# Kodifly/FAST-LIO-SAM_GPS

Measured on AMD Instinct MI355X. Metric: scans/sec (100k-pt scan vs N-pt map) + ms/IESKF-iteration, 1 GPU, higher is better.
Workload: dtype f32/f64; 1 GPU; C3: 131072-pt livox scan vs 5000000-pt map grown by 20 scans (map_incremental), max_iteration=3 (<=4 h-evals/scan); scan_points=131072, map_points=5000000, resident_scans=8, parallelism=replicas x1 (front end does not shard)

## Files before the change

fast-lio-sam_gps_amd/csrc/ieskf.cpp:

```cpp
#include "ieskf.hpp"

#include <chrono>
#include <cmath>
#include <cstring>

namespace lio {
namespace host {

namespace {

constexpr double kTol = 1e-11;
constexpr double kGravLen = 98090.0 / 10000.0;
constexpr int kSO3[2] = {3, 6};
constexpr int kS2 = 21;

Quat qmul(const Quat& a, const Quat& b) {
    return {a.w * b.w - a.x * b.x - a.y * b.y - a.z * b.z, a.w * b.x + a.x * b.w + a.y * b.z - a.z * b.y,
            a.w * b.y + a.y * b.w + a.z * b.x - a.x * b.z, a.w * b.z + a.z * b.w + a.x * b.y - a.y * b.x};
}

Quat qexp(const double* v, double h) {
    const double nrm = std::sqrt(v[0] * v[0] + v[1] * v[1] + v[2] * v[2]);
    if (nrm < kTol) return {1.0, h * v[0], h * v[1], h * v[2]};
    const double a = h * nrm, s = std::sin(a) / nrm;
// ... 126 lines not shown
    qlog(qmul(oc, x.offR), d + 6);
    for (int i = 0; i < 3; ++i) {
        d[9 + i] = x.offT[i] - y.offT[i];
        d[12 + i] = x.vel[i] - y.vel[i];
        d[15 + i] = x.bg[i] - y.bg[i];
        d[18 + i] = x.ba[i] - y.ba[i];
    }
    s2_minus(x.grav, y.grav, d + 21);
}

void boxplus(State& x, const double* d) {
    for (int i = 0; i < 3; ++i) x.pos[i] += d[i];
    x.rot = qmul(x.rot, qexp(d + 3, 0.5));
    x.offR = qmul(x.offR, qexp(d + 6, 0.5));
    for (int i = 0; i < 3; ++i) {
        x.offT[i] += d[9 + i];
        x.vel[i] += d[12 + i];
        x.bg[i] += d[15 + i];
        x.ba[i] += d[18 + i];
    }
    s2_plus(x.grav, d + 21);
}

bool lu_inverse(Mat& A, int n) {
    std::vector<int> piv(n);
    Mat LU = A;
    for (int k = 0; k < n; ++k) {
        int p = k;
        double best = std::fabs(LU[(size_t)k * n + k]);
        for (int r = k + 1; r < n; ++r) {
            const double v = std::fabs(LU[(size_t)r * n + k]);
            if (v > best) {
                best = v;
                p = r;
            }
        }
        piv[k] = p;
        if (best == 0.0) return false;
        if (p != k)
            for (int c = 0; c < n; ++c) std::swap(LU[(size_t)k * n + c], LU[(size_t)p * n + c]);
        const double inv = 1.0 / LU[(size_t)k * n + k];
        for (int r = k + 1; r < n; ++r) {
            const double f = (LU[(size_t)r * n + k] *= inv);
            if (f != 0.0)
                for (int c = k + 1; c < n; ++c) LU[(size_t)r * n + c] -= f * LU[(size_t)k * n + c];
        }
    }
    Mat X((size_t)n * n, 0.0);
    std::vector<double> col(n);
    for (int j = 0; j < n; ++j) {
        for (int i = 0; i < n; ++i) col[i] = (i == j) ? 1.0 : 0.0;
        for (int k = 0; k < n; ++k)
            if (piv[k] != k) std::swap(col[k], col[piv[k]]);
        for (int i = 0; i < n; ++i) {
            double s = col[i];
            for (int k = 0; k < i; ++k) s -= LU[(size_t)i * n + k] * col[k];
            col[i] = s;
        }
        for (int i = n - 1; i >= 0; --i) {
            double s = col[i];
            for (int k = i + 1; k < n; ++k) s -= LU[(size_t)i * n + k] * col[k];
            col[i] = s / LU[(size_t)i * n + i];
        }
        for (int i = 0; i < n; ++i) X[(size_t)i * n + j] = col[i];
    }
    A.swap(X);
    return true;
}

void rows_apply(Mat& Dst, const Mat& Src, int stride, int idx, const double* T, int d, int ncols) {
    double tmp[3];
    for (int c = 0; c < ncols; ++c) {
        for (int r = 0; r < d; ++r) {
            double s = 0;
            for (int k = 0; k < d; ++k) s += T[r * d + k] * Src[(size_t)(idx + k) * stride + c];
            tmp[r] = s;
        }
        for (int r = 0; r < d; ++r) Dst[(size_t)(idx + r) * stride + c] = tmp[r];
    }
}
void cols_apply(Mat& M, int nrows, int stride, int idx, const double* T, int d) {
    double tmp[3];
    for (int r = 0; r < nrows; ++r) {
        double* row = &M[(size_t)r * stride + idx];
        for (int c = 0; c < d; ++c) {
            double s = 0;
            for (int k = 0; k < d; ++k) s += row[k] * T[c * d + k];
            tmp[c] = s;
        }
// ... 13 lines not shown

}

void quat_to_mat(const Quat& q, double R[9]) {
    const double tx = 2 * q.x, ty = 2 * q.y, tz = 2 * q.z;
    const double twx = tx * q.w, twy = ty * q.w, twz = tz * q.w;
    const double txx = tx * q.x, txy = ty * q.x, txz = tz * q.x;
    const double tyy = ty * q.y, tyz = tz * q.y, tzz = tz * q.z;
    R[0] = 1 - (tyy + tzz);
    R[1] = txy - twz;
    R[2] = txz + twy;
    R[3] = txy + twz;
    R[4] = 1 - (txx + tzz);
    R[5] = tyz - twx;
    R[6] = txz - twy;
    R[7] = tyz + twx;
    R[8] = 1 - (txx + tyy);
}

int update_iterated(State& x, Mat& P, double R, int max_iter, double epsi, const HModelFn& hfn, IeskfResult& out) {
    using clk = std::chrono::steady_clock;
    const State x_prop = x;
    const Mat P_prop = P;
    Mat K_x((size_t)N * N, 0.0), Mm(36);
    double K_h[N], dx_new[N], dxu[N];
    bool converge = true;
    int t = 0;
    HModel hm;
    out = IeskfResult{};
    double solve_s = 0.0;
    for (int i = -1; i < max_iter; ++i) {
        const bool want_rows_hint = false;
        ++out.h_evals;
        if (converge) ++out.knn_calls;
        int rc = hfn(x, converge, want_rows_hint, hm);
        if (rc != 0) return rc;
        const int dof = (int)hm.sums[27];
        out.n_eff = dof;
        out.res_mean = dof > 0 ? hm.sums[28] / dof : 0.0;
        if (dof < 1) continue;
        if (dof < N && hm.rows.size() != (size_t)7 * dof) {
            rc = hfn(x, false, true, hm);
            if (rc != 0) return rc;
        }
        const auto t0 = clk::now();
        double dx[N];
        boxminus(x, x_prop, dx);
        std::memcpy(dx_new, dx, sizeof(dx));
// ... 13 lines not shown
            const double v1 = T2[2] * dx_new[kS2] + T2[3] * dx_new[kS2 + 1];
            dx_new[kS2] = v0;
            dx_new[kS2 + 1] = v1;
            rows_apply(P, P, N, kS2, T2, 2, N);
            cols_apply(P, N, N, kS2, T2, 2);
        }
        std::fill(K_x.begin(), K_x.end(), 0.0);
        if (N > dof) {
            const double* H = hm.rows.data();
            Mat PHt((size_t)N * dof);
            for (int r = 0; r < N; ++r)
                for (int m = 0; m < dof; ++m) {
                    double s = 0;
                    for (int c = 0; c < 6; ++c) s += P[(size_t)r * N + c] * H[7 * m + c];
                    PHt[(size_t)r * dof + m] = s;
                }
            Mat S((size_t)dof * dof);
            for (int a = 0; a < dof; ++a)
                for (int b = 0; b < dof; ++b) {
                    double s = 0;
                    for (int c = 0; c < 6; ++c) s += H[7 * a + c] * PHt[(size_t)c * dof + b];
                    S[(size_t)a * dof + b] = s / R + (a == b ? 1.0 : 0.0);
                }
            if (!lu_inverse(S, dof)) return -4;
            for (int r = 0; r < N; ++r) {
                double kh = 0;
                double kx[6] = {0, 0, 0, 0, 0, 0};
                for (int b = 0; b < dof; ++b) {
                    double s = 0;
                    for (int a = 0; a < dof; ++a) s += PHt[(size_t)r * dof + a] * S[(size_t)a * dof + b];
                    const double k = s / R;
                    kh += k * H[7 * b + 6];
                    for (int c = 0; c < 6; ++c) kx[c] += k * H[7 * b + c];
                }
                K_h[r] = kh;
                for (int c = 0; c < 6; ++c) K_x[(size_t)r * N + c] = kx[c];
            }
        } else {
            double HTH[36];
            unpack_hth(hm.sums, HTH);
            double PR[N * 6];
            for (int r = 0; r < N; ++r)
                for (int m = 0; m < 6; ++m) PR[r * 6 + m] = P[(size_t)r * N + m] / R;
            Mm.assign(36, 0.0);
            for (int a = 0; a < 6; ++a)
                for (int b = 0; b < 6; ++b) {
                    double s = 0;
                    for (int m = 0; m < 6; ++m) s += HTH[6 * a + m] * PR[m * 6 + b];
                    Mm[(size_t)a * 6 + b] = s + (a == b ? 1.0 : 0.0);
                }
            if (!lu_inverse(Mm, 6)) return -4;
            for (int r = 0; r < N; ++r) {
                double q[6];
                for (int c = 0; c < 6; ++c) {
                    double s = 0;
                    for (int m = 0; m < 6; ++m) s += PR[r * 6 + m] * Mm[(size_t)m * 6 + c];
                    q[c] = s;
                }
                double kh = 0;
                for (int c = 0; c < 6; ++c) kh += q[c] * hm.sums[21 + c];
                K_h[r] = kh;
                for (int c = 0; c < 6; ++c) {
                    double s = 0;
                    for (int m = 0; m < 6; ++m) s += q[m] * HTH[6 * m + c];
                    K_x[(size_t)r * N + c] = s;
                }
            }
        }
        for (int r = 0; r < N; ++r) {
            double s = 0;
            for (int c = 0; c < 6; ++c) s += (K_x[(size_t)r * N + c] - (r == c ? 1.0 : 0.0)) * dx_new[c];
            if (r >= 6) s += -dx_new[r];
            dxu[r] = K_h[r] + s;
        }
        boxplus(x, dxu);
        converge = true;
        for (int r = 0; r < N; ++r)
            if (std::fabs(dxu[r]) > epsi) {
                converge = false;
                break;
            }
        if (converge) ++t;
        if (!t && i == max_iter - 2) converge = true;
        if (t > 1 || i == max_iter - 1) {
            Mat L = P;
            for (int idx : kSO3) {
                const M3 At = transpose(a_matrix(dxu + idx));
                rows_apply(L, P, N, idx, At.a, 3, N);
                rows_apply(K_x, K_x, N, idx, At.a, 3, 12);
                cols_apply(L, N, N, idx, At.a, 3);
                cols_apply(P, N, N, idx, At.a, 3);
            }
            {
                double T2[4];
                s2_jac(x.grav, x_prop.grav, dxu + kS2, T2);
                rows_apply(L, P, N, kS2, T2, 2, N);
                rows_apply(K_x, K_x, N, kS2, T2, 2, 12);
                cols_apply(L, N, N, kS2, T2, 2);
                cols_apply(P, N, N, kS2, T2, 2);
            }
            Mat Pn((size_t)N * N);
            for (int r = 0; r < N; ++r)
                for (int c = 0; c < N; ++c) {
                    double s = 0;
                    for (int m = 0; m < 6; ++m) s += K_x[(size_t)r * N + m] * P[(size_t)m * N + c];
                    Pn[(size_t)r * N + c] = L[(size_t)r * N + c] - s;
                }
            P.swap(Pn);
            out.converged = t > 1 ? 1 : 0;
            solve_s += std::chrono::duration<double>(clk::now() - t0).count();
            break;
        }
        solve_s += std::chrono::duration<double>(clk::now() - t0).count();
    }
    out.solve_ms = solve_s * 1e3;
    return 0;
}

}
}
```

fast-lio-sam_gps_amd/csrc/lio_capi_online.hpp:

```cpp
#pragma once
#include <atomic>
#include <cmath>

#include "lio_capi_util.hpp"
#include "lio_mapupd.hpp"

struct lio_map : lio::capi::Handle {
    uint64_t version = 0;
    std::atomic<int> n_ctx{0};
    lio_map_params p{};
    lio::GridBuf grid;
    lio::MapUpdBuf upd;
    float* d_xyz = nullptr;
    int64_t xyz_cap = 0;
    int64_t n = 0;
    int32_t* d_qidx = nullptr;
    int64_t qidx_cap = 0;
    float* d_qd2 = nullptr;
    int64_t qd2_cap = 0;
};

namespace lio::capi {
struct EventPair {
    hipEvent_t a = nullptr, b = nullptr;
// ... 1 lines not shown
}

struct lio_ctx {
    lio_map* map = nullptr;
    double last_launch_ms = 0.0, last_wait_ms = 0.0;
    lio_match_params p{};
    int64_t n = 0, cap = 0;
    float* d_body = nullptr;
    const float* body_ext = nullptr;
    int32_t* d_nn = nullptr;
    float4* d_planes = nullptr;
    uint8_t* d_sel = nullptr;
    double* d_partials = nullptr;
    int64_t part_cap = 0;
    double* d_sums = nullptr;
    double* h_sums = nullptr;
    double* h_sums_dev = nullptr;
    unsigned long long seq = 0;
    double* d_rows = nullptr;
    int64_t rows_cap = 0;
    int64_t* d_nrows = nullptr;
    lio_pose last_pose{};
    lio_pose knn_pose{};
    int* d_far_list = nullptr;
    int* d_far_count = nullptr;
    unsigned* d_done = nullptr;
    float* d_far_d = nullptr;
    int* d_far_id = nullptr;
    float* d_d5 = nullptr;
    float* d_dbg = nullptr;
    int64_t dbg_cap = 0;
    bool have_eval = false;
    bool knn_valid = false;
    uint64_t knn_map_version = 0;
    bool timing = false;
    lio_kernel_timing tm{};
    lio::capi::EventPair ev_main, ev_fin;
    hipEvent_t ev_marks[8] = {};
    lio::FilterBuf filt;
    float* d_raw = nullptr;
    int64_t raw_cap = 0;
    float* d_rec = nullptr;
    int64_t rec_cap = 0;
    lio::ImuPose* d_poses = nullptr;
    int64_t poses_cap = 0;
    float seed_scale = 1.0f;
    int64_t undist_n = -1;
    int undist_stride = 0;
    float* d_kf = nullptr;
    int64_t kf_cap = 0;
};
// ... 56 lines not shown
```

fast-lio-sam_gps_amd/csrc/lio_capi_scan.cpp:

```cpp
#include <algorithm>
#include <chrono>
#include <cmath>
#include <cstring>
#include <string>

#include "ieskf.hpp"
#include "lio_capi_online.hpp"

using namespace lio::capi;

static void ctx_free(lio_ctx& c) {
    lio::dev_free(&c.d_body, &c.d_nn, &c.d_planes, &c.d_sel, &c.d_partials, &c.d_sums, &c.d_rows, &c.d_nrows,
                  &c.d_far_list, &c.d_far_count, &c.d_far_d, &c.d_far_id, &c.d_done, &c.d_d5, &c.d_dbg, &c.d_raw,
                  &c.d_rec, &c.d_poses, &c.d_kf);
    lio::host_free(&c.h_sums);
    for (hipEvent_t* e : {&c.ev_main.a, &c.ev_main.b, &c.ev_fin.a, &c.ev_fin.b})
        if (*e) (void)hipEventDestroy(*e);
    for (hipEvent_t e : c.ev_marks)
        if (e) (void)hipEventDestroy(e);
    lio::filter_free(c.filt);
}

int lio::capi::ctx_reserve(lio_ctx* c, int64_t n) {
    if (n > c->cap || !c->d_body) {
        const int64_t cap = std::max<int64_t>(n, c->cap + c->cap / 2);
        c->cap = 0;
        if (lio::dev_alloc_all({lio::dev_req(c->d_body, cap * 3), lio::dev_req(c->d_nn, cap * 5),
                                lio::dev_req(c->d_planes, cap), lio::dev_req(c->d_sel, cap + 64),
                                lio::dev_req(c->d_far_list, cap), lio::dev_req(c->d_far_d, cap * 5),
                                lio::dev_req(c->d_far_id, cap * 5), lio::dev_req(c->d_d5, cap)}))
            return fail(LIO_ERR_NOMEM, "scan buffers: hipMalloc failed");
        c->cap = cap;
    }
    int rc = grow(&c->d_partials, c->part_cap, (int64_t)lio::match_blocks((int)n) * 32 + 32);
    if (rc) return rc;
    c->n = n;
    c->body_ext = nullptr;
    c->have_eval = false;
    c->knn_valid = false;
    return LIO_OK;
}

extern "C" {

int lio_ctx_create(lio_map* m, const lio_match_params* p, lio_ctx** out) {
    if (!m || !out) return fail(LIO_ERR_ARG, "bad arguments");
    HIP_TRY(hipSetDevice(m->dev));
    auto* c = new lio_ctx();
    c->map = m;
    ++m->n_ctx;
    if (p)
        c->p = *p;
    else
        c->p = lio_match_params{5.0f, 0.1f, 0.9, 0.9};
    if (hipMalloc(&c->d_sums, 32 * sizeof(double)) != hipSuccess ||
        hipHostMalloc(&c->h_sums, 40 * sizeof(double), hipHostMallocMapped | hipHostMallocCoherent) != hipSuccess ||
        hipHostGetDevicePointer(reinterpret_cast<void**>(&c->h_sums_dev), c->h_sums, 0) != hipSuccess ||
// ... 45 lines not shown
}

int lio_scan_bind_device(lio_ctx* c, const float* d_body, int64_t n) {
    if (!c || n < 0 || (n > 0 && !d_body) || n >= (int64_t)1 << 30) return fail(LIO_ERR_ARG, "lio_scan_bind_device: bad arguments");
    HIP_TRY(hipSetDevice(c->map->dev));
    int rc = ctx_reserve(c, n);
    if (rc) return rc;
    c->body_ext = n ? d_body : nullptr;
    return LIO_OK;
}

static_assert(sizeof(lio_pose) == sizeof(lio::PoseArg), "lio_pose / PoseArg layout");

static lio::MatchArgs make_args(lio_ctx* c, const lio_pose& pose_in) {
    lio::MatchArgs a{};
    const lio_pose pose = filled(pose_in);
    std::memcpy(&a.pose, &pose, sizeof(lio::PoseArg));
    a.grid = lio::grid_view(c->map->grid);
    a.body = body_ptr(c);
    a.map_by_id = c->map->grid.by_id;
    a.nn_idx = c->d_nn;
    a.nn_d5 = c->d_d5;
    a.seed_scale = c->seed_scale;
    {
        const lio_pose pk = filled(c->knn_pose);
        std::memcpy(&a.pose_knn, &pk, sizeof(lio::PoseArg));
        double R[9], RL[9];
        quat_to_mat(pk.q, R);
        quat_to_mat(pk.q_LI, RL);
        for (int r = 0; r < 3; ++r) {
            for (int k = 0; k < 3; ++k)
                a.knn_M[4 * r + k] =
                    (float)(R[3 * r] * RL[k] + R[3 * r + 1] * RL[3 + k] + R[3 * r + 2] * RL[6 + k]);
            a.knn_M[4 * r + 3] =
                (float)(R[3 * r] * pk.t_LI[0] + R[3 * r + 1] * pk.t_LI[1] + R[3 * r + 2] * pk.t_LI[2] + pk.t[r]);
        }
    }
    a.planes = c->d_planes;
    a.sel = c->d_sel;
    a.partials = c->d_partials;
    a.n = (int)c->n;
    a.max_shell = (int)std::ceil(std::sqrt((double)c->p.knn_range_sq) / a.grid.cell) + 1;
    a.dbg = nullptr;
    a.sums_out = c->h_sums_dev;
    a.seq_out = reinterpret_cast<unsigned long long*>(c->h_sums_dev + 32);
    a.seq = 0;
    a.far_list = c->d_far_list;
    a.far_count = c->d_far_count;
    a.done_count = c->d_done;
    a.far_d = c->d_far_d;
    a.far_id = c->d_far_id;
    a.range_sq = c->p.knn_range_sq;
    a.plane_thr = c->p.plane_thr;
    a.s_coef = c->p.s_coef;
    a.s_gate = c->p.s_gate;
    return a;
}

static void accum_event(EventPair& e, int64_t& launches, double& ms) {
    float t = 0.f;
    if (hipEventElapsedTime(&t, e.a, e.b) == hipSuccess) {
        ms += t;
        ++launches;
    }
}

static uint64_t mix64(uint64_t z) {
    z = (z ^ (z >> 30)) * 0xbf58476d1ce4e5b9ull;
    z = (z ^ (z >> 27)) * 0x94d049bb133111ebull;
    return z ^ (z >> 31);
}

static bool read_result(const lio_ctx* c, unsigned long long seq, double* sums) {
    const volatile uint64_t* w = reinterpret_cast<const volatile uint64_t*>(c->h_sums);
    if (w[32] != seq) return false;
    uint64_t h = 0, bits[LIO_SUMS_LEN];
    for (int l = 0; l < LIO_SUMS_LEN; ++l) {
        bits[l] = w[l];
        h ^= mix64(bits[l] ^ ((uint64_t)l * 0x9e3779b97f4a7c15ull));
    }
    if ((h ^ mix64(seq)) != w[33]) return false;
    std::memcpy(sums, bits, sizeof(bits));
    return true;
}

static int wait_result(lio_ctx* c, unsigned long long seq, double* sums) {
    for (uint64_t it = 0;; ++it) {
        if (read_result(c, seq, sums)) return LIO_OK;
        if ((it & 255) == 255) {
            const hipError_t e = hipStreamQuery(c->map->st);
            if (e != hipSuccess && e != hipErrorNotReady)
                return fail(LIO_ERR_HIP, std::string("lio_match: ") + hipGetErrorString(e));
            if (e == hipSuccess && !read_result(c, seq, sums))
                return fail(LIO_ERR_HIP, "lio_match: evaluation produced no result");
        }
    }
}

static int match_impl(lio_ctx* c, const lio_pose* pose_in, int redo_knn, double* sums);

int lio_match(lio_ctx* c, const lio_pose* pose_in, int redo_knn, double* sums) {
    if (!c || !pose_in || !sums) return fail(LIO_ERR_ARG, "lio_match: bad arguments");
    return match_impl(c, pose_in, redo_knn, sums);
}

static int match_impl(lio_ctx* c, const lio_pose* pose_in, int redo_knn, double* sums) {
    const lio_pose pose_f = filled(*pose_in);
    const lio_pose* pose = &pose_f;
    if (c->map->grid.n_ids == 0) return fail(LIO_ERR_STATE, "lio_match: map is empty (call lio_map_build)");
    if (!redo_knn && !c->knn_valid) return fail(LIO_ERR_STATE, "lio_match: redo_knn=0 before any kNN evaluation");
    if (!redo_knn && c->knn_map_version != c->map->version)
        return fail(LIO_ERR_STATE, "lio_match: redo_knn=0 but the map changed since this scan's kNN evaluation");
    HIP_TRY(hipSetDevice(c->map->dev));
    hipStream_t st = c->map->st;
    lio::MatchArgs a = make_args(c, *pose);
    if (c->map->n == 0 && c->n > 0) {
        HIP_TRY(hipMemsetAsync(c->d_nn, 0xff, c->n * 5 * sizeof(int32_t), st));
        HIP_TRY(hipMemsetAsync(c->d_sel, 0, c->n, st));
        HIP_TRY(hipStreamSynchronize(st));
    }
    if (c->n == 0 || c->map->n == 0) {
        std::memset(sums, 0, LIO_SUMS_LEN * sizeof(double));
        c->last_pose = *pose;
        c->have_eval = true;
        c->knn_valid = true;
        c->knn_map_version = c->map->version;
        c->knn_pose = *pose;
        return LIO_OK;
    }
    a.seq = ++c->seq;
    a.prior = (redo_knn && c->knn_valid && c->knn_map_version == c->map->version) ? 1 : 0;
    const auto t0 = std::chrono::steady_clock::now();
    if (c->timing) HIP_TRY(hipEventRecord(c->ev_main.a, st));
    lio::launch_h_model(a, redo_knn != 0, st, c->timing ? c->ev_marks : nullptr);
    if (c->timing) HIP_TRY(hipEventRecord(c->ev_main.b, st));
    HIP_TRY(hipGetLastError());
    const auto t1 = std::chrono::steady_clock::now();
    int rc = wait_result(c, a.seq, sums);
    if (rc) return rc;
    const auto t2 = std::chrono::steady_clock::now();
    c->last_launch_ms = std::chrono::duration<double, std::milli>(t1 - t0).count();
    c->last_wait_ms = std::chrono::duration<double, std::milli>(t2 - t1).count();
    if (c->timing) {
        HIP_TRY(hipEventSynchronize(c->ev_main.b));
        if (redo_knn) {
            const double before = c->tm.near_ms + c->tm.far_ms + c->tm.plane_ms;
            EventPair n{c->ev_marks[0], c->ev_marks[1]}, f{c->ev_marks[2], c->ev_marks[3]},
                p{c->ev_marks[4], c->ev_marks[5]};
            accum_event(n, c->tm.near_launches, c->tm.near_ms);
            if (a.max_shell > 1) accum_event(f, c->tm.far_launches, c->tm.far_ms);
            accum_event(p, c->tm.plane_launches, c->tm.plane_ms);
            c->tm.knn_ms += (c->tm.near_ms + c->tm.far_ms + c->tm.plane_ms) - before;
            ++c->tm.knn_launches;
        } else {
            EventPair r{c->ev_marks[6], c->ev_marks[7]};
            accum_event(r, c->tm.reuse_launches, c->tm.reuse_ms);
        }
    }
    c->last_pose = *pose;
    c->have_eval = true;
    if (redo_knn) {
        c->knn_valid = true;
        c->knn_map_version = c->map->version;
        c->knn_pose = *pose;
    }
    return LIO_OK;
}

int lio_ctx_knn_stats(lio_ctx* c, const lio_pose* pose, double* sums, int32_t* stats3) {
    if (!c || !pose || !sums || !stats3) return fail(LIO_ERR_ARG, "lio_ctx_knn_stats: bad arguments");
    if (c->map->n == 0) return fail(LIO_ERR_STATE, "lio_ctx_knn_stats: map is empty");
    HIP_TRY(hipSetDevice(c->map->dev));
    hipStream_t st = c->map->st;
    if (c->n == 0) return LIO_OK;
    static_assert(sizeof(int) == sizeof(float), "the debug scratch holds either");
    int rc = grow(&c->d_dbg, c->dbg_cap, c->n * 3);
    if (rc) return rc;
    lio::MatchArgs a = make_args(c, *pose);
    a.dbg = reinterpret_cast<int*>(c->d_dbg);
    a.seq = ++c->seq;
    lio::launch_h_model(a, true, st);
    hipError_t e2 = hipMemcpyAsync(stats3, c->d_dbg, c->n * 3 * sizeof(int), hipMemcpyDeviceToHost, st);
    hipError_t e3 = hipStreamSynchronize(st);
    if (e2 != hipSuccess || e3 != hipSuccess) return fail(LIO_ERR_HIP, "lio_ctx_knn_stats failed");
    rc = wait_result(c, a.seq, sums);
    if (rc) return rc;
    c->last_pose = *pose;
    c->knn_pose = *pose;
    c->have_eval = true;
    c->knn_valid = true;
    c->knn_map_version = c->map->version;
    return LIO_OK;
}

int lio_ctx_get_knn_pose(lio_ctx* c, lio_pose* out) {
    if (!c || !out) return fail(LIO_ERR_ARG, "bad arguments");
    if (!c->knn_valid) return fail(LIO_ERR_STATE, "lio_ctx_get_knn_pose: no kNN evaluation");
    *out = c->knn_pose;
    return LIO_OK;
}

int lio_map_incremental(lio_ctx* c, const lio_pose* pose, double filter_size_map, lio_incremental_stats* st) {
    if (!c || !pose || !(filter_size_map > 0.0)) return fail(LIO_ERR_ARG, "lio_map_incremental: bad arguments");
    if (c->n > 0 && !c->knn_valid && c->map->n > 0)
        return fail(LIO_ERR_STATE, "lio_map_incremental: no kNN evaluation for this scan (Nearest_Points)");
    if (c->n > 0 && c->map->n > 0 && c->knn_map_version != c->map->version)
        return fail(LIO_ERR_STATE, "lio_map_incremental: the map changed since this scan's kNN evaluation");
    lio_map* m = c->map;
// ... 200 lines not shown
```

fast-lio-sam_gps_amd/csrc/lio_dev.hpp:

```cpp
#pragma once
#include <hip/hip_runtime.h>
#include <stdint.h>

namespace lio {

constexpr int kNone = 0x7fffffff;

struct GridDev {
    const float4* pts;
    const uint32_t* start;
    const uint2* rng;
    float ox, oy, oz;
    float cell, inv_cell;
    float margin;
    int nx, ny, nz;
};

struct PoseArg {
    double R[9];
    double t[3];
    double RLI[9];
    double tLI[3];
    double q[4];
    double qLI[4];
// ... 122 lines not shown
    float g = fmaxf(fmaxf(lo - q, q - hi), 0.f);
    return g * g;
}

template <int OFF>
__device__ __forceinline__ uint32_t partner_u32(uint32_t v) {
    if constexpr (OFF == 1) return (uint32_t)__builtin_amdgcn_update_dpp((int)v, (int)v, 0xb1, 0xf, 0xf, false);
    else if constexpr (OFF == 2) return (uint32_t)__builtin_amdgcn_update_dpp((int)v, (int)v, 0x4e, 0xf, 0xf, false);
    else if constexpr (OFF == 4) return (uint32_t)__builtin_amdgcn_update_dpp((int)v, (int)v, 0x141, 0xf, 0xf, false);
    else return (uint32_t)__shfl_xor((int)v, OFF, 64);
}
template <int OFF>
__device__ __forceinline__ float partner_f(float v) {
    return __uint_as_float(partner_u32<OFF>(__float_as_uint(v)));
}

template <int G, int OFF = 1>
__device__ __forceinline__ float group_min(float v) {
    if constexpr (OFF >= G) {
        return v;
    } else {
        v = fminf(v, partner_f<OFF>(v));
        return group_min<G, 2 * OFF>(v);
    }
}

template <int K>
__device__ __forceinline__ void cmpx(uint64_t (&v)[K], int i, int j) {
    const uint64_t a = v[i], b = v[j];
    v[i] = key_min(a, b);
    v[j] = key_max(a, b);
}
template <int K>
__device__ __forceinline__ void sort_bitonic(uint64_t (&v)[K]) {
    static_assert(K == 1 || K == 5, "sort_bitonic: K = 1 or 5");
    if constexpr (K == 5) {
        cmpx(v, 0, 4);
        cmpx(v, 1, 3);
        cmpx(v, 1, 4);
        cmpx(v, 2, 4);
        cmpx(v, 3, 4);
    }
}

template <int K, int G, int OFF = 1>
__device__ __forceinline__ void group_merge(TopK<K>& tk) {
// ... 302 lines not shown
    float own = fminf(fminf(qx - lox, lox + cs - qx), fminf(qy - loy, loy + cs - qy));
    own = fminf(own, fminf(qz - loz, loz + cs - qz)) - m;
    const uint32_t nx = (uint32_t)g.nx, nxy = (uint32_t)g.nx * (uint32_t)g.ny;
    const uint32_t c0 = (uint32_t)cz * nxy + (uint32_t)cy * nx + (uint32_t)cx;
    uint32_t b4[shell1_cpl<G>()], n4[shell1_cpl<G>()];
    shell1_ranges<G>(g, cx, cy, cz, sub, b4, n4);
    scan_cell_group2<K, G, UO>(g, c0, qx, qy, qz, sub, tk);
    group_merge<K, G>(tk);
    if (dbg) dbg->shell = 0;
    if (own > 0.f && tk.worst() < own * own * 0.999999f) return true;
    if (sub != 0) {
        tk.fill_with_worst();
    }
    scan_shell1_flat<K, G, U>(g, qx, qy, qz, cx, cy, cz, lox, loy, loz, sub, lds, b4, n4, tk, dbg);
    group_merge<K, G>(tk);
    if (dbg) dbg->shell = 1;
    const float gr = own + cs;
    if (gr > 0.f && tk.worst() < gr * gr * 0.999999f) return true;
    if (!TAIL || max_shell < 2) return false;
    if (dbg) dbg->shell = 2;
    return group_knn_exact_from<K, G>(g, qx, qy, qz, 2, max_shell, sub, tk);
}

__device__ __forceinline__ float seeded_bound(bool inside, float d5prev, float wox, float woy, float woz, float qx,
                                             float qy, float qz, float range_sq, float scale) {
    float bound = range_sq;
    if (inside && d5prev <= range_sq) {
        const float dx = qx - wox, dy = qy - woy, dz = qz - woz;
        const float eps = 1e-4f + 1e-6f * ((fabsf(qx) + fabsf(qy)) + fabsf(qz));
        const float r = (sqrtf(d5prev) + sqrtf((dx * dx + dy * dy) + dz * dz)) + eps;
        const float b = r * r * (1.0f + 1e-5f);
        if (b < range_sq) bound = b * scale;
    }
    return bound;
}

template <int K, int G, int U = 4>
__device__ int group_knn_seeded(const GridDev& g, float bound, int cx, int cy, int cz, float qx, float qy, float qz,
                                 float range_sq, int sub, TopK<K>& tk, uint32_t* lds) {
    static_assert(K == 5, "group_knn_seeded: K = 5");
    const bool inside = (unsigned)cx < (unsigned)g.nx && (unsigned)cy < (unsigned)g.ny && (unsigned)cz < (unsigned)g.nz;
    tk.init(bound);
    if (!inside) return 0;
    uint32_t b4[shell1_cpl<G>()], n4[shell1_cpl<G>()];
    shell1_ranges<G, true>(g, cx, cy, cz, sub, b4, n4);
    const float cs = g.cell, m = g.margin;
    const float lox = g.ox + (float)cx * cs, loy = g.oy + (float)cy * cs, loz = g.oz + (float)cz * cs;
    float own = fminf(fminf(qx - lox, lox + cs - qx), fminf(qy - loy, loy + cs - qy));
    own = fminf(own, fminf(qz - loz, loz + cs - qz)) - m;
    const uint32_t TP = shell1_table<K, G>(g, qx, qy, qz, lox, loy, loz, sub, lds, b4, n4, tk.worst(), nullptr);
    __builtin_amdgcn_fence(__ATOMIC_RELEASE, "wavefront");
    __builtin_amdgcn_wave_barrier();
    __builtin_amdgcn_fence(__ATOMIC_ACQUIRE, "wavefront");
    scan_table_strided<K, U>(g, qx, qy, qz, lds, TP & 0xffffffu, TP >> 24, (uint32_t)sub, (uint32_t)G, tk);
    group_merge<K, G>(tk);
    if (tk.id(K - 1) == kNone && bound < range_sq) {
// ... 466 lines not shown
```

fast-lio-sam_gps_amd/csrc/lio_kernels.hpp:

```cpp
#pragma once
#include <hip/hip_runtime.h>
#include <stdint.h>

#include "lio_dev.hpp"

namespace lio {

struct MatchArgs {
    PoseArg pose;
    GridDev grid;
    const float* body;
    const float4* map_by_id;
    int32_t* nn_idx;
    float* nn_d5;
    float4* planes;
    uint8_t* sel;
    double* partials;
    double* sums_out;
    unsigned long long* seq_out;
    unsigned long long seq;
    int* dbg;
    int* far_list;
    int* far_count;
    unsigned* done_count;
    float* far_d;
    int* far_id;
    int n;
    int max_shell;
    int prior;
    float range_sq;
    float plane_thr;
    double s_coef;
    double s_gate;
    PoseArg pose_knn;
    float knn_M[12];
    float seed_scale;
};

int launch_h_model(const MatchArgs& a, bool redo, hipStream_t st, hipEvent_t* marks = nullptr);
void launch_debug(const MatchArgs& a, float* world, float* d2, float* abcd_pd2, hipStream_t st);
void launch_h_rows(const MatchArgs& a, double* rows, int64_t max_rows, int64_t* n_rows, hipStream_t st);
int match_blocks(int n);
void launch_map_knn(const GridDev& g, const float* q, int n, float bound, int max_shell, int k, int32_t* idx,
                    float* d2, hipStream_t st);

struct GridGeom {
    float ox, oy, oz, cell;
    int nx, ny, nz;
    uint32_t ncells;
};

struct GridBuf {
    float4* pts = nullptr;
    uint32_t* ckeys = nullptr;
    float4* by_id = nullptr;
    uint32_t* start = nullptr;
    int64_t n = 0, cap = 0;
    int64_t n_ids = 0, id_cap = 0;
    uint32_t cells_cap = 0;
    GridGeom geom{};
    bool gapped = false;
    uint2* rng = nullptr;
    uint32_t* lim = nullptr;
    uint32_t* addc = nullptr;
    uint8_t* dirty = nullptr;
// ... 84 lines not shown
```

fast-lio-sam_gps_amd/csrc/lio_match.hip:

```cpp
#include <hip/hip_ext.h>

#include "lio_dev.hpp"
#include "lio_kernels.hpp"

#include <algorithm>

namespace lio {

constexpr int kBlock = 256;
constexpr int kPlaneBlock = 512;
constexpr int kReuseBlock = 512;
constexpr int kReusePpl = 2;
constexpr int kNearBlock = 256;

constexpr int kGroup = 8;
constexpr int kFarBlock = 128;
constexpr int kFarBlocks = 1024;

__device__ __forceinline__ double wave_sum(double v) {
#pragma unroll
    for (int off = 32; off > 0; off >>= 1) v += __shfl_xor(v, off, 64);
    return v;
}

__device__ __forceinline__ bool residual_row(const MatchArgs& a, const PoseArg& ps, float bx, float by, float bz, float wx, float wy,
                                             float wz, const float4& pl, double J[6], double& h, double& res) {
    const float pd2 = ((pl.x * wx + pl.y * wy) + pl.z * wz) + pl.w;
    const double b0 = bx, b1 = by, b2 = bz;
    const double pn = sqrt((b0 * b0 + b1 * b1) + b2 * b2);
    const float s = (float)(1.0 - a.s_coef * (double)fabsf(pd2) / sqrt(pn));
    if (!((double)s > a.s_gate)) return false;
    h_row(ps, bx, by, bz, pl.x, pl.y, pl.z, J);
    h = -(double)pd2;
    res = (double)fabsf(pd2);
    return true;
}

template <bool DBG, bool SEEDED, int U, int NB, int UO>
__global__ void __launch_bounds__(NB) __attribute__((amdgpu_waves_per_eu(8, 8))) knn_near_kernel(MatchArgs a) {
    const PoseArg& ps = a.pose;
    constexpr int G = kGroup;
    constexpr int QPB = NB / G;
    __shared__ uint32_t s_tab[QPB][72];
    __shared__ float s_q[4][QPB];
    __shared__ int s_c[3][QPB];
    const int blk = xcd_block(blockIdx.x, gridDim.x);
    const int sub = threadIdx.x % G;
    const int q = threadIdx.x / G;
    const int i = blk * QPB + q;
    if (threadIdx.x < QPB) {
        const int iq = blk * QPB + (int)threadIdx.x;
        if (iq < a.n) {
            const float bx = a.body[3 * iq], by = a.body[3 * iq + 1], bz = a.body[3 * iq + 2];
            float wx, wy, wz;
            body_to_world(ps, bx, by, bz, wx, wy, wz);
            s_q[0][threadIdx.x] = wx;
            s_q[1][threadIdx.x] = wy;
            s_q[2][threadIdx.x] = wz;
            const int cx = cell_coord(wx, a.grid.ox, a.grid.inv_cell);
            const int cy = cell_coord(wy, a.grid.oy, a.grid.inv_cell);
            const int cz = cell_coord(wz, a.grid.oz, a.grid.inv_cell);
            s_c[0][threadIdx.x] = cx;
            s_c[1][threadIdx.x] = cy;
            s_c[2][threadIdx.x] = cz;
            if constexpr (SEEDED) {
                const float* M = a.knn_M;
                const float wox = ((M[0] * bx + M[1] * by) + M[2] * bz) + M[3];
                const float woy = ((M[4] * bx + M[5] * by) + M[6] * bz) + M[7];
                const float woz = ((M[8] * bx + M[9] * by) + M[10] * bz) + M[11];
                const bool inside = (unsigned)cx < (unsigned)a.grid.nx && (unsigned)cy < (unsigned)a.grid.ny &&
                                    (unsigned)cz < (unsigned)a.grid.nz;
                s_q[3][threadIdx.x] = seeded_bound(inside, a.nn_d5[iq], wox, woy, woz, wx, wy, wz, a.range_sq, a.seed_scale);
            }
        }
    }
    __syncthreads();
    if (i >= a.n) return;
    const float wx = s_q[0][q], wy = s_q[1][q], wz = s_q[2][q];
    TopK<5> tk;
    tk.init(a.range_sq);
    SearchStats st{0, 0, 0};
    bool done, whole = false;
    if constexpr (SEEDED) {
        const int r = group_knn_seeded<5, G, U>(a.grid, s_q[3][q], s_c[0][q], s_c[1][q], s_c[2][q], wx, wy, wz, a.range_sq, sub,
                                                tk, s_tab[threadIdx.x / G]);
        done = r > 0;
        whole = r < 0;
    } else {
        done = group_knn_near<5, G, false, U, UO>(a.grid, wx, wy, wz, s_c[0][q], s_c[1][q], s_c[2][q], 1, sub, tk,
                                              DBG ? &st : nullptr, s_tab[threadIdx.x / G]);
    }
    const bool far = !done && a.max_shell > 1;
    if constexpr (DBG) {
#pragma unroll
        for (int off = 1; off < G; off <<= 1) {
            st.cells += __shfl_xor(st.cells, off, 64);
            st.points += __shfl_xor(st.points, off, 64);
        }
        if (sub == 0) {
            a.dbg[3 * (size_t)i] = st.cells;
            a.dbg[3 * (size_t)i + 1] = st.points;
            a.dbg[3 * (size_t)i + 2] = far ? 2 : st.shell;
        }
    }
    if (far) {
        if (sub == 0) {
            const int slot = atomicAdd(a.far_count, 1);
            a.far_list[slot] = whole ? (int)((unsigned)i | 0x80000000u) : i;
#pragma unroll
            for (int j = 0; j < 5; ++j) {
                a.far_d[5 * (size_t)slot + j] = tk.d(j);
                a.far_id[5 * (size_t)slot + j] = tk.id(j);
            }
        }
        return;
    }
#pragma unroll
    for (int js = 0; js < 5; js += G) {
        const int jj = js + sub;
        if (jj < 5) {
            int v = tk.id(0);
#pragma unroll
            for (int j = 1; j < 5; ++j)
                if (jj == j) v = tk.id(j);
            a.nn_idx[5 * (size_t)i + jj] = v == kNone ? -1 : v;
        }
    }
    if (sub == 5) a.nn_d5[i] = tk.id(4) == kNone ? INFINITY : tk.d(4);
}

template <int NT = kFarBlock>
__global__ void __launch_bounds__(NT) knn_far_kernel(MatchArgs a) {
    const PoseArg& ps = a.pose;
    __shared__ uint32_t s_b[NT], s_off[NT + 1], s_w[NT / 64];
    __shared__ uint64_t s_lists[(NT / 64) * 5];
    const int cnt = *a.far_count;
    for (int f = blockIdx.x; f < cnt; f += gridDim.x) {
        const int e = a.far_list[f];
        const int i = e & 0x7fffffff;
        float wx, wy, wz;
        body_to_world(ps, a.body[3 * i], a.body[3 * i + 1], a.body[3 * i + 2], wx, wy, wz);
        TopK<5> tk;
#pragma unroll
        for (int j = 0; j < 5; ++j) tk.k[j] = knn_key(a.far_d[5 * (size_t)f + j], a.far_id[5 * (size_t)f + j]);
        block_knn_box_flat<5, NT>(a.grid, wx, wy, wz, s_b, s_off, s_w, s_lists, tk, e < 0);
        if (threadIdx.x == 0) {
#pragma unroll
            for (int j = 0; j < 5; ++j) a.nn_idx[5 * (size_t)i + j] = tk.id(j) == kNone ? -1 : tk.id(j);
            a.nn_d5[i] = tk.id(4) == kNone ? INFINITY : tk.d(4);
        }
    }
}

typedef __attribute__((address_space(1))) double gdouble;
typedef __attribute__((address_space(1))) unsigned int guint;
typedef __attribute__((address_space(1))) unsigned long long gull;

__device__ __forceinline__ unsigned long long mix64(unsigned long long z) {
    z = (z ^ (z >> 30)) * 0xbf58476d1ce4e5b9ull;
    z = (z ^ (z >> 27)) * 0x94d049bb133111ebull;
    return z ^ (z >> 31);
}

__device__ __forceinline__ void publish_host(double t, double* out, unsigned long long* seq_out, unsigned long long seq) {
    const int lane = threadIdx.x & 63;
    unsigned long long h =
        lane < 32 ? mix64((unsigned long long)__double_as_longlong(t) ^ ((unsigned long long)lane * 0x9e3779b97f4a7c15ull))
                  : 0ull;
#pragma unroll
    for (int off = 1; off < 32; off <<= 1) h ^= __shfl_xor(h, off, 64);
    h = __shfl(h, 0, 64);
    if (lane < 32) __hip_atomic_store((gdouble*)(out + lane), t, __ATOMIC_RELAXED, __HIP_MEMORY_SCOPE_SYSTEM);
    else if (lane == 32) __hip_atomic_store((gull*)seq_out, seq, __ATOMIC_RELAXED, __HIP_MEMORY_SCOPE_SYSTEM);
// ... 303 lines not shown
        return nbp;
    }
    const int nbr = (a.n + kReusePpl * kReuseBlock - 1) / (kReusePpl * kReuseBlock);
    hipExtLaunchKernelGGL((h_model_reuse_kernel<kReusePpl, kReuseBlock>), dim3(nbr), dim3(kReuseBlock), 0, st, m[6],
                          m[7], 0, a);
    return nbr;
}

void launch_debug(const MatchArgs& a, float* world, float* d2, float* abcd_pd2, hipStream_t st) {
    if (a.n == 0) return;
    debug_kernel<<<(a.n + 255) / 256, 256, 0, st>>>(a, world, d2, abcd_pd2);
}

void launch_h_rows(const MatchArgs& a, double* rows, int64_t max_rows, int64_t* n_rows, hipStream_t st) {
    h_rows_kernel<<<1, 1024, 0, st>>>(a, rows, max_rows, n_rows);
}

void launch_map_knn(const GridDev& g, const float* q, int n, float bound, int max_shell, int k, int32_t* idx,
                    float* d2, hipStream_t st) {
    if (n <= 0) return;
    map_knn_kernel<<<(n + 256 / kGroup - 1) / (256 / kGroup), 256, 0, st>>>(g, q, n, bound, max_shell, k, idx, d2);
}

int match_blocks(int n) {
    return (n + kBlock - 1) / kBlock;
}

}
```

Measured before the change: 5833 scans/s.

## Pack far-queue entries, derive seeded bounds from previous neighbours, throttle stream polling

```diff
diff --git a/fast-lio-sam_gps_amd/csrc/ieskf.cpp b/fast-lio-sam_gps_amd/csrc/ieskf.cpp
--- a/fast-lio-sam_gps_amd/csrc/ieskf.cpp
+++ b/fast-lio-sam_gps_amd/csrc/ieskf.cpp
@@ -172,9 +172,10 @@
     s2_plus(x.grav, d + 21);
 }
 
-bool lu_inverse(Mat& A, int n) {
-    std::vector<int> piv(n);
-    Mat LU = A;
+bool lu_inverse(double* A, int n) {
+    int piv[N];
+    double LU[N * N], X[N * N], col[N];
+    std::memcpy(LU, A, sizeof(double) * (size_t)n * n);
     for (int k = 0; k < n; ++k) {
         int p = k;
         double best = std::fabs(LU[(size_t)k * n + k]);
@@ -196,8 +197,6 @@
                 for (int c = k + 1; c < n; ++c) LU[(size_t)r * n + c] -= f * LU[(size_t)k * n + c];
         }
     }
-    Mat X((size_t)n * n, 0.0);
-    std::vector<double> col(n);
     for (int j = 0; j < n; ++j) {
         for (int i = 0; i < n; ++i) col[i] = (i == j) ? 1.0 : 0.0;
         for (int k = 0; k < n; ++k)
@@ -214,7 +213,7 @@
         }
         for (int i = 0; i < n; ++i) X[(size_t)i * n + j] = col[i];
     }
-    A.swap(X);
+    std::memcpy(A, X, sizeof(double) * (size_t)n * n);
     return true;
 }
 
@@ -274,8 +273,8 @@
     using clk = std::chrono::steady_clock;
     const State x_prop = x;
     const Mat P_prop = P;
-    Mat K_x((size_t)N * N, 0.0), Mm(36);
-    double K_h[N], dx_new[N], dxu[N];
+    Mat K_x((size_t)N * N, 0.0), L((size_t)N * N), Pn((size_t)N * N);
+    double K_h[N], dx_new[N], dxu[N], Mm[36];
     bool converge = true;
     int t = 0;
     HModel hm;
@@ -335,7 +334,7 @@
                     for (int c = 0; c < 6; ++c) s += H[7 * a + c] * PHt[(size_t)c * dof + b];
                     S[(size_t)a * dof + b] = s / R + (a == b ? 1.0 : 0.0);
                 }
-            if (!lu_inverse(S, dof)) return -4;
+            if (!lu_inverse(S.data(), dof)) return -4;
             for (int r = 0; r < N; ++r) {
                 double kh = 0;
                 double kx[6] = {0, 0, 0, 0, 0, 0};
@@ -355,7 +354,6 @@
             double PR[N * 6];
             for (int r = 0; r < N; ++r)
                 for (int m = 0; m < 6; ++m) PR[r * 6 + m] = P[(size_t)r * N + m] / R;
-            Mm.assign(36, 0.0);
             for (int a = 0; a < 6; ++a)
                 for (int b = 0; b < 6; ++b) {
                     double s = 0;
@@ -396,7 +394,7 @@
         if (converge) ++t;
         if (!t && i == max_iter - 2) converge = true;
         if (t > 1 || i == max_iter - 1) {
-            Mat L = P;
+            L = P;
             for (int idx : kSO3) {
                 const M3 At = transpose(a_matrix(dxu + idx));
                 rows_apply(L, P, N, idx, At.a, 3, N);
@@ -412,7 +410,6 @@
                 cols_apply(L, N, N, kS2, T2, 2);
                 cols_apply(P, N, N, kS2, T2, 2);
             }
-            Mat Pn((size_t)N * N);
             for (int r = 0; r < N; ++r)
                 for (int c = 0; c < N; ++c) {
                     double s = 0;
diff --git a/fast-lio-sam_gps_amd/csrc/lio_capi_online.hpp b/fast-lio-sam_gps_amd/csrc/lio_capi_online.hpp
--- a/fast-lio-sam_gps_amd/csrc/lio_capi_online.hpp
+++ b/fast-lio-sam_gps_amd/csrc/lio_capi_online.hpp
@@ -47,11 +47,10 @@
     int64_t* d_nrows = nullptr;
     lio_pose last_pose{};
     lio_pose knn_pose{};
-    int* d_far_list = nullptr;
+    lio::FarEntry* d_far_q = nullptr;
+    int64_t far_cap = 0;
     int* d_far_count = nullptr;
     unsigned* d_done = nullptr;
-    float* d_far_d = nullptr;
-    int* d_far_id = nullptr;
     float* d_d5 = nullptr;
     float* d_dbg = nullptr;
     int64_t dbg_cap = 0;
diff --git a/fast-lio-sam_gps_amd/csrc/lio_capi_scan.cpp b/fast-lio-sam_gps_amd/csrc/lio_capi_scan.cpp
--- a/fast-lio-sam_gps_amd/csrc/lio_capi_scan.cpp
+++ b/fast-lio-sam_gps_amd/csrc/lio_capi_scan.cpp
@@ -11,7 +11,7 @@
 
 static void ctx_free(lio_ctx& c) {
     lio::dev_free(&c.d_body, &c.d_nn, &c.d_planes, &c.d_sel, &c.d_partials, &c.d_sums, &c.d_rows, &c.d_nrows,
-                  &c.d_far_list, &c.d_far_count, &c.d_far_d, &c.d_far_id, &c.d_done, &c.d_d5, &c.d_dbg, &c.d_raw,
+                  &c.d_far_q, &c.d_far_count, &c.d_done, &c.d_d5, &c.d_dbg, &c.d_raw,
                   &c.d_rec, &c.d_poses, &c.d_kf);
     lio::host_free(&c.h_sums);
     for (hipEvent_t* e : {&c.ev_main.a, &c.ev_main.b, &c.ev_fin.a, &c.ev_fin.b})
@@ -27,12 +27,13 @@
         c->cap = 0;
         if (lio::dev_alloc_all({lio::dev_req(c->d_body, cap * 3), lio::dev_req(c->d_nn, cap * 5),
                                 lio::dev_req(c->d_planes, cap), lio::dev_req(c->d_sel, cap + 64),
-                                lio::dev_req(c->d_far_list, cap), lio::dev_req(c->d_far_d, cap * 5),
-                                lio::dev_req(c->d_far_id, cap * 5), lio::dev_req(c->d_d5, cap)}))
+                                lio::dev_req(c->d_d5, cap)}))
             return fail(LIO_ERR_NOMEM, "scan buffers: hipMalloc failed");
         c->cap = cap;
     }
     int rc = grow(&c->d_partials, c->part_cap, (int64_t)lio::match_blocks((int)n) * 32 + 32);
+    if (rc) return rc;
+    rc = grow(&c->d_far_q, c->far_cap, lio::far_entries(n));
     if (rc) return rc;
     c->n = n;
     c->body_ext = nullptr;
@@ -124,20 +125,6 @@
     a.nn_idx = c->d_nn;
     a.nn_d5 = c->d_d5;
     a.seed_scale = c->seed_scale;
-    {
-        const lio_pose pk = filled(c->knn_pose);
-        std::memcpy(&a.pose_knn, &pk, sizeof(lio::PoseArg));
-        double R[9], RL[9];
-        quat_to_mat(pk.q, R);
-        quat_to_mat(pk.q_LI, RL);
-        for (int r = 0; r < 3; ++r) {
-            for (int k = 0; k < 3; ++k)
-                a.knn_M[4 * r + k] =
-                    (float)(R[3 * r] * RL[k] + R[3 * r + 1] * RL[3 + k] + R[3 * r + 2] * RL[6 + k]);
-            a.knn_M[4 * r + 3] =
-                (float)(R[3 * r] * pk.t_LI[0] + R[3 * r + 1] * pk.t_LI[1] + R[3 * r + 2] * pk.t_LI[2] + pk.t[r]);
-        }
-    }
     a.planes = c->d_planes;
     a.sel = c->d_sel;
     a.partials = c->d_partials;
@@ -147,11 +134,9 @@
     a.sums_out = c->h_sums_dev;
     a.seq_out = reinterpret_cast<unsigned long long*>(c->h_sums_dev + 32);
     a.seq = 0;
-    a.far_list = c->d_far_list;
+    a.far_q = c->d_far_q;
     a.far_count = c->d_far_count;
     a.done_count = c->d_done;
-    a.far_d = c->d_far_d;
-    a.far_id = c->d_far_id;
     a.range_sq = c->p.knn_range_sq;
     a.plane_thr = c->p.plane_thr;
     a.s_coef = c->p.s_coef;
@@ -186,16 +171,20 @@
     return true;
 }
 
-static int wait_result(lio_ctx* c, unsigned long long seq, double* sums) {
+static int wait_result(lio_ctx* c, unsigned long long seq, double* sums, std::chrono::steady_clock::time_point launched) {
+    constexpr std::chrono::microseconds kFirstQuery{80}, kQueryPeriod{50};
+    auto next = launched + kFirstQuery;
     for (uint64_t it = 0;; ++it) {
         if (read_result(c, seq, sums)) return LIO_OK;
-        if ((it & 255) == 255) {
-            const hipError_t e = hipStreamQuery(c->map->st);
-            if (e != hipSuccess && e != hipErrorNotReady)
-                return fail(LIO_ERR_HIP, std::string("lio_match: ") + hipGetErrorString(e));
-            if (e == hipSuccess && !read_result(c, seq, sums))
-                return fail(LIO_ERR_HIP, "lio_match: evaluation produced no result");
-        }
+        if ((it & 63) != 63) continue;
+        const auto now = std::chrono::steady_clock::now();
+        if (now < next) continue;
+        next = now + kQueryPeriod;
+        const hipError_t e = hipStreamQuery(c->map->st);
+        if (e != hipSuccess && e != hipErrorNotReady)
+            return fail(LIO_ERR_HIP, std::string("lio_match: ") + hipGetErrorString(e));
+        if (e == hipSuccess && !read_result(c, seq, sums))
+            return fail(LIO_ERR_HIP, "lio_match: evaluation produced no result");
     }
 }
 
@@ -238,7 +227,7 @@
     if (c->timing) HIP_TRY(hipEventRecord(c->ev_main.b, st));
     HIP_TRY(hipGetLastError());
     const auto t1 = std::chrono::steady_clock::now();
-    int rc = wait_result(c, a.seq, sums);
+    int rc = wait_result(c, a.seq, sums, t1);
     if (rc) return rc;
     const auto t2 = std::chrono::steady_clock::now();
     c->last_launch_ms = std::chrono::duration<double, std::milli>(t1 - t0).count();
@@ -285,7 +274,7 @@
     hipError_t e2 = hipMemcpyAsync(stats3, c->d_dbg, c->n * 3 * sizeof(int), hipMemcpyDeviceToHost, st);
     hipError_t e3 = hipStreamSynchronize(st);
     if (e2 != hipSuccess || e3 != hipSuccess) return fail(LIO_ERR_HIP, "lio_ctx_knn_stats failed");
-    rc = wait_result(c, a.seq, sums);
+    rc = wait_result(c, a.seq, sums, std::chrono::steady_clock::now());
     if (rc) return rc;
     c->last_pose = *pose;
     c->knn_pose = *pose;
diff --git a/fast-lio-sam_gps_amd/csrc/lio_dev.hpp b/fast-lio-sam_gps_amd/csrc/lio_dev.hpp
--- a/fast-lio-sam_gps_amd/csrc/lio_dev.hpp
+++ b/fast-lio-sam_gps_amd/csrc/lio_dev.hpp
@@ -168,6 +168,16 @@
     } else {
         v = fminf(v, partner_f<OFF>(v));
         return group_min<G, 2 * OFF>(v);
+    }
+}
+
+template <int G, int OFF = 1>
+__device__ __forceinline__ float group_max(float v) {
+    if constexpr (OFF >= G) {
+        return v;
+    } else {
+        v = fmaxf(v, partner_f<OFF>(v));
+        return group_max<G, 2 * OFF>(v);
     }
 }
 
@@ -516,16 +526,9 @@
     return group_knn_exact_from<K, G>(g, qx, qy, qz, 2, max_shell, sub, tk);
 }
 
-__device__ __forceinline__ float seeded_bound(bool inside, float d5prev, float wox, float woy, float woz, float qx,
-                                             float qy, float qz, float range_sq, float scale) {
+__device__ __forceinline__ float seeded_bound(bool inside, float b, float range_sq, float scale) {
     float bound = range_sq;
-    if (inside && d5prev <= range_sq) {
-        const float dx = qx - wox, dy = qy - woy, dz = qz - woz;
-        const float eps = 1e-4f + 1e-6f * ((fabsf(qx) + fabsf(qy)) + fabsf(qz));
-        const float r = (sqrtf(d5prev) + sqrtf((dx * dx + dy * dy) + dz * dz)) + eps;
-        const float b = r * r * (1.0f + 1e-5f);
-        if (b < range_sq) bound = b * scale;
-    }
+    if (inside && b < range_sq) bound = b * scale;
     return bound;
 }
 
diff --git a/fast-lio-sam_gps_amd/csrc/lio_kernels.hpp b/fast-lio-sam_gps_amd/csrc/lio_kernels.hpp
--- a/fast-lio-sam_gps_amd/csrc/lio_kernels.hpp
+++ b/fast-lio-sam_gps_amd/csrc/lio_kernels.hpp
@@ -5,6 +5,14 @@
 #include "lio_dev.hpp"
 
 namespace lio {
+
+struct alignas(64) FarEntry {
+    int32_t i;
+    float w[3];
+    uint64_t k[5];
+    uint64_t pad;
+};
+static_assert(sizeof(FarEntry) == 64, "FarEntry: one 64-byte line per queued query");
 
 struct MatchArgs {
     PoseArg pose;
@@ -20,11 +28,9 @@
     unsigned long long* seq_out;
     unsigned long long seq;
     int* dbg;
-    int* far_list;
+    FarEntry* far_q;
     int* far_count;
     unsigned* done_count;
-    float* far_d;
-    int* far_id;
     int n;
     int max_shell;
     int prior;
@@ -32,8 +38,6 @@
     float plane_thr;
     double s_coef;
     double s_gate;
-    PoseArg pose_knn;
-    float knn_M[12];
     float seed_scale;
 };
 
@@ -41,6 +45,7 @@
 void launch_debug(const MatchArgs& a, float* world, float* d2, float* abcd_pd2, hipStream_t st);
 void launch_h_rows(const MatchArgs& a, double* rows, int64_t max_rows, int64_t* n_rows, hipStream_t st);
 int match_blocks(int n);
+int64_t far_entries(int64_t n);
 void launch_map_knn(const GridDev& g, const float* q, int n, float bound, int max_shell, int k, int32_t* idx,
                     float* d2, hipStream_t st);
 
diff --git a/fast-lio-sam_gps_amd/csrc/lio_match.hip b/fast-lio-sam_gps_amd/csrc/lio_match.hip
--- a/fast-lio-sam_gps_amd/csrc/lio_match.hip
+++ b/fast-lio-sam_gps_amd/csrc/lio_match.hip
@@ -42,37 +42,32 @@
     constexpr int G = kGroup;
     constexpr int QPB = NB / G;
     __shared__ uint32_t s_tab[QPB][72];
-    __shared__ float s_q[4][QPB];
+    __shared__ float s_q[3][QPB];
     __shared__ int s_c[3][QPB];
     const int blk = xcd_block(blockIdx.x, gridDim.x);
     const int sub = threadIdx.x % G;
     const int q = threadIdx.x / G;
     const int i = blk * QPB + q;
-    if (threadIdx.x < QPB) {
-        const int iq = blk * QPB + (int)threadIdx.x;
-        if (iq < a.n) {
-            const float bx = a.body[3 * iq], by = a.body[3 * iq + 1], bz = a.body[3 * iq + 2];
-            float wx, wy, wz;
-            body_to_world(ps, bx, by, bz, wx, wy, wz);
-            s_q[0][threadIdx.x] = wx;
-            s_q[1][threadIdx.x] = wy;
-            s_q[2][threadIdx.x] = wz;
-            const int cx = cell_coord(wx, a.grid.ox, a.grid.inv_cell);
-            const int cy = cell_coord(wy, a.grid.oy, a.grid.inv_cell);
-            const int cz = cell_coord(wz, a.grid.oz, a.grid.inv_cell);
-            s_c[0][threadIdx.x] = cx;
-            s_c[1][threadIdx.x] = cy;
-            s_c[2][threadIdx.x] = cz;
-            if constexpr (SEEDED) {
-                const float* M = a.knn_M;
-                const float wox = ((M[0] * bx + M[1] * by) + M[2] * bz) + M[3];
-                const float woy = ((M[4] * bx + M[5] * by) + M[6] * bz) + M[7];
-                const float woz = ((M[8] * bx + M[9] * by) + M[10] * bz) + M[11];
-                const bool inside = (unsigned)cx < (unsigned)a.grid.nx && (unsigned)cy < (unsigned)a.grid.ny &&
-                                    (unsigned)cz < (unsigned)a.grid.nz;
-                s_q[3][threadIdx.x] = seeded_bound(inside, a.nn_d5[iq], wox, woy, woz, wx, wy, wz, a.range_sq, a.seed_scale);
-            }
-        }
+    const int iq = blk * QPB + (int)threadIdx.x;
+    const bool lead = threadIdx.x < QPB && iq < a.n;
+    float bx, by, bz;
+    if (lead) bx = a.body[3 * iq], by = a.body[3 * iq + 1], bz = a.body[3 * iq + 2];
+    int pid = -1;
+    float4 pp = make_float4(0.f, 0.f, 0.f, 0.f);
+    if constexpr (SEEDED) {
+        if (sub < 5 && i < a.n) pid = a.nn_idx[5 * (size_t)i + sub];
+        if (pid >= 0) pp = a.map_by_id[pid];
+    }
+    if (lead) {
+        asm volatile("" : "+v"(bx), "+v"(by), "+v"(bz));
+        float wx, wy, wz;
+        body_to_world(ps, bx, by, bz, wx, wy, wz);
+        s_q[0][threadIdx.x] = wx;
+        s_q[1][threadIdx.x] = wy;
+        s_q[2][threadIdx.x] = wz;
+        s_c[0][threadIdx.x] = cell_coord(wx, a.grid.ox, a.grid.inv_cell);
+        s_c[1][threadIdx.x] = cell_coord(wy, a.grid.oy, a.grid.inv_cell);
+        s_c[2][threadIdx.x] = cell_coord(wz, a.grid.oz, a.grid.inv_cell);
     }
     __syncthreads();
     if (i >= a.n) return;
@@ -82,7 +77,13 @@
     SearchStats st{0, 0, 0};
     bool done, whole = false;
     if constexpr (SEEDED) {
-        const int r = group_knn_seeded<5, G, U>(a.grid, s_q[3][q], s_c[0][q], s_c[1][q], s_c[2][q], wx, wy, wz, a.range_sq, sub,
+        const int cx = s_c[0][q], cy = s_c[1][q], cz = s_c[2][q];
+        const bool inside = (unsigned)cx < (unsigned)a.grid.nx && (unsigned)cy < (unsigned)a.grid.ny &&
+                            (unsigned)cz < (unsigned)a.grid.nz;
+        float d = sub < 5 ? INFINITY : 0.f;
+        if (pid >= 0) d = sqdist3(wx, wy, wz, pp.x, pp.y, pp.z);
+        const float bound = seeded_bound(inside, group_max<G>(d), a.range_sq, a.seed_scale);
+        const int r = group_knn_seeded<5, G, U>(a.grid, bound, cx, cy, cz, wx, wy, wz, a.range_sq, sub,
                                                 tk, s_tab[threadIdx.x / G]);
         done = r > 0;
         whole = r < 0;
@@ -106,12 +107,13 @@
     if (far) {
         if (sub == 0) {
             const int slot = atomicAdd(a.far_count, 1);
-            a.far_list[slot] = whole ? (int)((unsigned)i | 0x80000000u) : i;
-#pragma unroll
-            for (int j = 0; j < 5; ++j) {
-                a.far_d[5 * (size_t)slot + j] = tk.d(j);
-                a.far_id[5 * (size_t)slot + j] = tk.id(j);
-            }
+            FarEntry e;
+            e.i = whole ? (int)((unsigned)i | 0x80000000u) : i;
+            e.w[0] = wx, e.w[1] = wy, e.w[2] = wz;
+#pragma unroll
+            for (int j = 0; j < 5; ++j) e.k[j] = tk.k[j];
+            e.pad = 0;
+            a.far_q[slot] = e;
         }
         return;
     }
@@ -131,24 +133,25 @@
 
 template <int NT = kFarBlock>
 __global__ void __launch_bounds__(NT) knn_far_kernel(MatchArgs a) {
-    const PoseArg& ps = a.pose;
     __shared__ uint32_t s_b[NT], s_off[NT + 1], s_w[NT / 64];
     __shared__ uint64_t s_lists[(NT / 64) * 5];
-    const int cnt = *a.far_count;
-    for (int f = blockIdx.x; f < cnt; f += gridDim.x) {
-        const int e = a.far_list[f];
-        const int i = e & 0x7fffffff;
-        float wx, wy, wz;
-        body_to_world(ps, a.body[3 * i], a.body[3 * i + 1], a.body[3 * i + 2], wx, wy, wz);
+    const FarEntry* __restrict__ fq = a.far_q;
+    FarEntry e = fq[blockIdx.x];
+    int cnt = *a.far_count;
+    asm volatile("" : "+s"(cnt), "+v"(e.i), "+v"(e.w[0]), "+v"(e.k[0]), "+v"(e.k[2]), "+v"(e.k[4]));
+    for (int f = blockIdx.x; f < cnt;) {
+        const int i = e.i & 0x7fffffff;
         TopK<5> tk;
 #pragma unroll
-        for (int j = 0; j < 5; ++j) tk.k[j] = knn_key(a.far_d[5 * (size_t)f + j], a.far_id[5 * (size_t)f + j]);
-        block_knn_box_flat<5, NT>(a.grid, wx, wy, wz, s_b, s_off, s_w, s_lists, tk, e < 0);
+        for (int j = 0; j < 5; ++j) tk.k[j] = e.k[j];
+        block_knn_box_flat<5, NT>(a.grid, e.w[0], e.w[1], e.w[2], s_b, s_off, s_w, s_lists, tk, e.i < 0);
         if (threadIdx.x == 0) {
 #pragma unroll
             for (int j = 0; j < 5; ++j) a.nn_idx[5 * (size_t)i + j] = tk.id(j) == kNone ? -1 : tk.id(j);
             a.nn_d5[i] = tk.id(4) == kNone ? INFINITY : tk.d(4);
         }
+        f += gridDim.x;
+        if (f < cnt) e = fq[f];
     }
 }
 
@@ -498,6 +501,10 @@
     map_knn_kernel<<<(n + 256 / kGroup - 1) / (256 / kGroup), 256, 0, st>>>(g, q, n, bound, max_shell, k, idx, d2);
 }
 
+int64_t far_entries(int64_t n) {
+    return std::max<int64_t>(n, kFarBlocks);
+}
+
 int match_blocks(int n) {
     return (n + kBlock - 1) / kBlock;
 }
```

New measurement: 6380 scans/s, median of 6. +9.4%, better.
